# facebookresearch/dmc-net

Measured on AMD Instinct MI355X. Metric: clips/sec (3-seg 224x224) DMC-gen+ResNet-18 train step, higher is better.
Workload: dtype f32

## Files before the change

dmc-net_amd/csrc/bn_act.hip:

```cpp
#include "dmc_common.h"

using namespace dmc;

namespace {

constexpr int MAX_SPLIT = BN_MAX_SPLIT;

struct BnArgs {
    const float* x;
    const float* res;
    const float* gamma;
    const float* beta;
    const float* stats;
    const float* dy;
    float* y;
    float* dx;
    float* dres;
    int M, C, relu;
    unsigned char* mask;
    const float* keep;
    int hw;
    float slope;
};

template <int MODE>
__global__ __launch_bounds__(256) void bn_partial_kernel(BnArgs a, double* __restrict__ scratch) {
    __shared__ double sm[2][256][4];
    const int cq = a.C >> 2;
    const int tx = threadIdx.x % cq, ty = threadIdx.x / cq, rows = 256 / cq;
    const int per = (a.M + (int)gridDim.x - 1) / (int)gridDim.x;
    const int r0 = blockIdx.x * per, r1 = (r0 + per < a.M) ? r0 + per : a.M;
    float4 s0 = make_float4(0.f, 0.f, 0.f, 0.f), s1 = s0;
    float4 mean = s0, istd = s0, g = s0, b = s0;
    if (MODE == 1) {
        mean = reinterpret_cast<const float4*>(a.stats)[tx];
        istd = reinterpret_cast<const float4*>(a.stats + a.C)[tx];
        g = reinterpret_cast<const float4*>(a.gamma)[tx];
        b = reinterpret_cast<const float4*>(a.beta)[tx];
    }
// ... 356 lines not shown
                                                           int M, int C, int hw, float slope) {
    const int cq = C >> 2;
    const size_t total = (size_t)M * cq;
    for (size_t o = (size_t)blockIdx.x * 256 + threadIdx.x; o < total; o += (size_t)gridDim.x * 256) {
        const int tx = (int)(o % cq);
        const float4 x = reinterpret_cast<const float4*>(z)[o];
        float4 d = reinterpret_cast<const float4*>(dz)[o];
        float4 k = make_float4(1.f, 1.f, 1.f, 1.f);
        if (keep) k = reinterpret_cast<const float4*>(keep)[(size_t)((o / cq) / hw) * cq + tx];
        d.x *= k.x * (x.x > 0.f ? 1.f : slope); d.y *= k.y * (x.y > 0.f ? 1.f : slope);
        d.z *= k.z * (x.z > 0.f ? 1.f : slope); d.w *= k.w * (x.w > 0.f ? 1.f : slope);
        reinterpret_cast<float4*>(dx)[o] = d;
    }
}

__global__ __launch_bounds__(256) void channel_sum_final_kernel(const double* __restrict__ scratch,
                                                                float* __restrict__ out, int C, int split) {
    const int c = blockIdx.x * 8 + (threadIdx.x >> 5), sub = threadIdx.x & 31;
    double s, ss;
    reduce_partials(scratch, C, c, split, sub, s, ss);
    if (c < C && sub == 0) out[c] = (float)s;
}

bool shape_ok(int M, int C) {
    const int cq = C / 4;
    return M > 0 && C > 0 && C % 4 == 0 && cq <= 256 && 256 % cq == 0;
}

int split_of(int M, int C) {
    long sp = (long)M * C / 8192;
    return sp < 1 ? 1 : (sp > MAX_SPLIT ? MAX_SPLIT : (int)sp);
}

int stream_blocks(size_t total) {
    size_t b = (total + 255) / 256;
    return (int)(b < 1 ? 1 : (b > 8192 ? 8192 : b));
}


__device__ __forceinline__ void load8(const float* p, size_t i8, float (&v)[8]) {
    const float4 a = reinterpret_cast<const float4*>(p)[2 * i8], b = reinterpret_cast<const float4*>(p)[2 * i8 + 1];
    v[0] = a.x; v[1] = a.y; v[2] = a.z; v[3] = a.w; v[4] = b.x; v[5] = b.y; v[6] = b.z; v[7] = b.w;
}
__device__ __forceinline__ void store8(float* p, size_t i8, const float (&v)[8]) {
    reinterpret_cast<float4*>(p)[2 * i8] = make_float4(v[0], v[1], v[2], v[3]);
    reinterpret_cast<float4*>(p)[2 * i8 + 1] = make_float4(v[4], v[5], v[6], v[7]);
}

__global__ __launch_bounds__(256) void bn_apply_fwd_x3s_kernel(BnArgs a, unsigned short* __restrict__ ys, int s2d_h, int s2d_w) {
    const int c8 = a.C >> 3;
    const size_t total = (size_t)a.M * c8;
    for (size_t o = (size_t)blockIdx.x * 256 + threadIdx.x; o < total; o += (size_t)gridDim.x * 256) {
        const int tx = (int)(o & (size_t)(c8 - 1));
        const size_t m = o / c8;
        float mean[8], istd[8], g[8], b[8], x[8], v[8];
        load8(a.stats, tx, mean); load8(a.stats + a.C, tx, istd); load8(a.gamma, tx, g); load8(a.beta, tx, b);
        load8(a.x, o, x);
#pragma unroll
        for (int e = 0; e < 8; ++e) v[e] = fmaf((x[e] - mean[e]) * istd[e], g[e], b[e]);
        if (a.res) {
            float rr[8];
            load8(a.res, o, rr);
#pragma unroll
            for (int e = 0; e < 8; ++e) v[e] += rr[e];
        }
        if (a.relu) {
// ... 24 lines not shown
                                                               const float* __restrict__ dbeta, float inv_count,
                                                               unsigned short* __restrict__ dxs) {
    const int c8 = a.C >> 3;
    const size_t total = (size_t)a.M * c8;
    for (size_t o = (size_t)blockIdx.x * 256 + threadIdx.x; o < total; o += (size_t)gridDim.x * 256) {
        const int tx = (int)(o & (size_t)(c8 - 1));
        const size_t m = o / c8;
        float mean[8], istd[8], g[8], b[8], dg[8], db[8], x[8], d[8], xh[8], r[8];
        load8(a.stats, tx, mean); load8(a.stats + a.C, tx, istd); load8(a.gamma, tx, g); load8(a.beta, tx, b);
        load8(dgamma, tx, dg); load8(dbeta, tx, db);
        load8(a.x, o, x); load8(a.dy, o, d);
#pragma unroll
        for (int e = 0; e < 8; ++e) xh[e] = (x[e] - mean[e]) * istd[e];
        if (a.relu && a.mask) {
            const unsigned mw = reinterpret_cast<const unsigned short*>(a.mask)[o];
            const unsigned mb = (mw & 15u) | ((mw >> 8) << 4);
#pragma unroll
            for (int e = 0; e < 8; ++e) d[e] = ((mb >> e) & 1u) ? d[e] : 0.f;
        } else if (a.relu) {
            float rr[8];
            if (a.res) load8(a.res, o, rr);
#pragma unroll
            for (int e = 0; e < 8; ++e) {
                float v = fmaf(xh[e], g[e], b[e]);
                if (a.res) v += rr[e];
                d[e] = v > 0.f ? d[e] : 0.f;
            }
        }
        if (a.dres) store8(a.dres, o, d);
#pragma unroll
        for (int e = 0; e < 8; ++e) r[e] = g[e] * istd[e] * (d[e] - db[e] * inv_count - xh[e] * dg[e] * inv_count);
        if (a.dx) store8(a.dx, o, r);
        if (dxs) x3s_store8(dxs, r, (size_t)a.M, a.C >> 4, m, tx);
    }
}

__global__ __launch_bounds__(256) void pool_fwd_x3s_kernel(PoolArgs a, unsigned short* __restrict__ ys, unsigned* __restrict__ codes,
                                                           float* __restrict__ xmax) {
    const int c8 = a.C >> 3;
    const size_t total = (size_t)a.N * a.PH * a.PW * c8;
    for (size_t o = (size_t)blockIdx.x * 256 + threadIdx.x; o < total; o += (size_t)gridDim.x * 256) {
        const int tx = (int)(o & (size_t)(c8 - 1));
        size_t r = o / c8;
        const size_t mp = r;
        const int px = (int)(r % a.PW); r /= a.PW;
        const int py = (int)(r % a.PH);
        const int n = (int)(r / a.PH);
        float mean[8], istd[8], g[8], b[8], mx[8];
        load8(a.stats, tx, mean); load8(a.stats + a.C, tx, istd); load8(a.gamma, tx, g); load8(a.beta, tx, b);
        float xv[9][8];
#pragma unroll
        for (int k = 0; k < 9; ++k) {
            int iy = 2 * py + k / 3 - 1, ix = 2 * px + k % 3 - 1;
            iy = iy < 0 ? 0 : (iy >= a.H ? a.H - 1 : iy);
            ix = ix < 0 ? 0 : (ix >= a.W ? a.W - 1 : ix);
            load8(a.x, ((size_t)(n * a.H + iy) * a.W + ix) * c8 + tx, xv[k]);
        }
        if (codes) {
            float bx[8];
            unsigned ck[8];
#pragma unroll
            for (int e = 0; e < 8; ++e) { mx[e] = -INFINITY; bx[e] = 0.f; ck[e] = 0; }
#pragma unroll
            for (int k = 0; k < 9; ++k) {
                const int iy = 2 * py + k / 3 - 1, ix = 2 * px + k % 3 - 1;
                const bool in = iy >= 0 && iy < a.H && ix >= 0 && ix < a.W;
#pragma unroll
                for (int e = 0; e < 8; ++e) {
                    const float v = fmaxf(fmaf((xv[k][e] - mean[e]) * istd[e], g[e], b[e]), 0.f);
                    const bool take = in && v > mx[e];
                    mx[e] = take ? v : mx[e];
                    bx[e] = take ? xv[k][e] : bx[e];
                    ck[e] = take ? (unsigned)k : ck[e];
                }
            }
            reinterpret_cast<uint2*>(codes)[o] = make_uint2(ck[0] | (ck[1] << 8) | (ck[2] << 16) | (ck[3] << 24),
                                                            ck[4] | (ck[5] << 8) | (ck[6] << 16) | (ck[7] << 24));
            store8(xmax, o, bx);
        } else {
#pragma unroll
            for (int e = 0; e < 8; ++e) mx[e] = 0.f;
#pragma unroll
            for (int k = 0; k < 9; ++k)
#pragma unroll
                for (int e = 0; e < 8; ++e) mx[e] = fmaxf(mx[e], fmaxf(fmaf((xv[k][e] - mean[e]) * istd[e], g[e], b[e]), 0.f));
        }
        if (a.ypool) store8(a.ypool, o, mx);
        if (ys) x3s_store8(ys, mx, (size_t)a.N * a.PH * a.PW, a.C >> 4, mp, tx);
    }
}

bool shape_ok8(int M, int C) { return shape_ok(M, C) && C % 16 == 0 && C >= 16; }

}

extern "C" {

int dmc_bn_act_supported(int M, int C) { return shape_ok(M, C) ? 1 : 0; }

size_t dmc_bn_act_stats_bytes(int C) { return (((size_t)2 * C * sizeof(float)) + 15) / 16 * 16; }
size_t dmc_bn_act_scratch_bytes(int C) { return (size_t)MAX_SPLIT * C * 2 * sizeof(double); }

int dmc_bn_act_fwd(const float* x, const float* residual, const float* gamma, const float* beta,
                   float* running_mean, float* running_var, float* y, float* stats, void* scratch_,
                   unsigned char* relu_mask, int M, int C, int relu, int training, float eps,
                   float momentum, dmc_stream_t stream) {
    if (!x || !gamma || !beta || !running_mean || !running_var || !y || !stats || (training && !scratch_))
        return fail(DMC_E_INVALID, "dmc_bn_act_fwd: null pointer");
    if (!shape_ok(M, C)) return fail(DMC_E_INVALID, "dmc_bn_act_fwd: unsupported shape M=%d C=%d", M, C);
    hipStream_t s = (hipStream_t)stream;
    BnArgs a = {x, residual, gamma, beta, stats, nullptr, y, nullptr, nullptr, M, C, relu, relu_mask};
    double* scratch = static_cast<double*>(scratch_);
    int rc;
    const int split = split_of(M, C);
    if (training) {
        bn_partial_kernel<0><<<split, 256, 0, s>>>(a, scratch);
        if ((rc = check_launch("bn_partial"))) return rc;
    }
    bn_stats_final_kernel<<<(C + 7) / 8, 256, 0, s>>>(scratch, stats, running_mean, running_var, C,
                                                       (long)M, training, eps, momentum, split);
    if ((rc = check_launch("bn_stats_final"))) return rc;
    bn_apply_fwd_kernel<<<stream_blocks((size_t)M * (C / 4)), 256, 0, s>>>(a);
    return check_launch("bn_apply_fwd");
}

int dmc_bn_act_bwd(const float* x, const float* residual, const float* gamma, const float* beta,
                   const float* stats, void* scratch_, const float* dy, float* dx, float* dresidual,
                   float* dgamma, float* dbeta, const unsigned char* relu_mask, int M, int C, int relu,
                   dmc_stream_t stream) {
    if (!x || !gamma || !beta || !stats || !scratch_ || !dy || !dx || !dgamma || !dbeta)
        return fail(DMC_E_INVALID, "dmc_bn_act_bwd: null pointer");
    if (!shape_ok(M, C)) return fail(DMC_E_INVALID, "dmc_bn_act_bwd: unsupported shape M=%d C=%d", M, C);
    hipStream_t s = (hipStream_t)stream;
    BnArgs a = {x, residual, gamma, beta, stats, dy, nullptr, dx, dresidual, M, C, relu,
                const_cast<unsigned char*>(relu_mask)};
    double* scratch = static_cast<double*>(scratch_);
    int rc;
    const int split = split_of(M, C);
    bn_partial_kernel<1><<<split, 256, 0, s>>>(a, scratch);
    if ((rc = check_launch("bn_bwd_partial"))) return rc;
    bn_bwd_final_kernel<<<C, 256, 0, s>>>(scratch, dgamma, dbeta, C, split);
    if ((rc = check_launch("bn_bwd_final"))) return rc;
    bn_apply_bwd_kernel<<<stream_blocks((size_t)M * (C / 4)), 256, 0, s>>>(a, dgamma, dbeta, 1.f / (float)M);
    return check_launch("bn_apply_bwd");
}

int dmc_bn_relu_pool_supported(int N, int H, int W, int C) {
    return N > 0 && H > 0 && W > 0 && shape_ok(1, C) && C / 4 <= 64 ? 1 : 0;
}

int dmc_bn_relu_pool_fwd(const float* x, const float* gamma, const float* beta, float* running_mean,
                         float* running_var, float* y_pool, float* stats, void* scratch_, int N, int H,
                         int W, int C, int training, float eps, float momentum, dmc_stream_t stream) {
    if (!x || !gamma || !beta || !running_mean || !running_var || !y_pool || !stats || (training && !scratch_))
        return fail(DMC_E_INVALID, "dmc_bn_relu_pool_fwd: null pointer");
    if (!dmc_bn_relu_pool_supported(N, H, W, C))
        return fail(DMC_E_INVALID, "dmc_bn_relu_pool_fwd: unsupported shape N=%d H=%d W=%d C=%d", N, H, W, C);
    hipStream_t s = (hipStream_t)stream;
    const int M = N * H * W;
    BnArgs a = {x, nullptr, gamma, beta, stats, nullptr, nullptr, nullptr, nullptr, M, C, 1, nullptr};
    double* scratch = static_cast<double*>(scratch_);
    int rc;
    const int split = split_of(M, C);
    if (training) {
        bn_partial_kernel<0><<<split, 256, 0, s>>>(a, scratch);
        if ((rc = check_launch("bn_partial"))) return rc;
    }
    bn_stats_final_kernel<<<(C + 7) / 8, 256, 0, s>>>(scratch, stats, running_mean, running_var, C,
                                                       (long)M, training, eps, momentum, split);
    if ((rc = check_launch("bn_stats_final"))) return rc;
    PoolArgs p = {x, gamma, beta, stats, nullptr, y_pool, nullptr, N, H, W, C, (H - 1) / 2 + 1, (W - 1) / 2 + 1};
    pool_fwd_kernel<<<stream_blocks((size_t)N * p.PH * p.PW * (C / 4)), 256, 0, s>>>(p);
// ... 78 lines not shown
    return check_launch("channel_sum_final");
}

int dmc_bn_apply_act_x3s(const float* x, const float* residual, const float* gamma, const float* beta, const float* stats,
                         float* y, void* ys, unsigned char* relu_mask, int M, int C, int relu, dmc_stream_t stream) {
    if (!x || !gamma || !beta || !stats || (!y && !ys)) return fail(DMC_E_INVALID, "dmc_bn_apply_act_x3s: null pointer");
    if (!shape_ok8(M, C)) return fail(DMC_E_INVALID, "dmc_bn_apply_act_x3s: unsupported shape M=%d C=%d", M, C);
    BnArgs a = {x, residual, gamma, beta, stats, nullptr, y, nullptr, nullptr, M, C, relu, relu_mask};
    bn_apply_fwd_x3s_kernel<<<stream_blocks((size_t)M * (C / 8)), 256, 0, (hipStream_t)stream>>>(a, static_cast<unsigned short*>(ys), 0, 0);
    return check_launch("bn_apply_act_x3s");
}

int dmc_bn_apply_act_x3q(const float* x, const float* residual, const float* gamma, const float* beta, const float* stats,
                         float* y, void* yq, unsigned char* relu_mask, int N, int H, int W, int C, int relu, dmc_stream_t stream) {
    if (!x || !gamma || !beta || !stats || !yq) return fail(DMC_E_INVALID, "dmc_bn_apply_act_x3q: null pointer");
    if (N <= 0 || H <= 0 || W <= 0 || (H & 1) || (W & 1) || (long)N * H * W >= (1L << 31)) return fail(DMC_E_INVALID, "dmc_bn_apply_act_x3q: bad geometry");
    const int M = N * H * W;
    if (!shape_ok8(M, C)) return fail(DMC_E_INVALID, "dmc_bn_apply_act_x3q: unsupported shape M=%d C=%d", M, C);
    BnArgs a = {x, residual, gamma, beta, stats, nullptr, y, nullptr, nullptr, M, C, relu, relu_mask};
    bn_apply_fwd_x3s_kernel<<<stream_blocks((size_t)M * (C / 8)), 256, 0, (hipStream_t)stream>>>(a, static_cast<unsigned short*>(yq), H, W);
    return check_launch("bn_apply_act_x3q");
}

int dmc_bn_act_bwd_x3s(const float* x, const float* residual, const float* gamma, const float* beta, const float* stats,
                       void* scratch_, const float* dy, float* dx, void* dxs, float* dresidual, float* dgamma, float* dbeta,
                       const unsigned char* relu_mask, int M, int C, int relu, dmc_stream_t stream) {
    if (!x || !gamma || !beta || !stats || !scratch_ || !dy || (!dx && !dxs) || !dgamma || !dbeta)
        return fail(DMC_E_INVALID, "dmc_bn_act_bwd_x3s: null pointer");
    if (!shape_ok8(M, C)) return fail(DMC_E_INVALID, "dmc_bn_act_bwd_x3s: unsupported shape M=%d C=%d", M, C);
    hipStream_t s = (hipStream_t)stream;
    BnArgs a = {x, residual, gamma, beta, stats, dy, nullptr, dx, dresidual, M, C, relu, const_cast<unsigned char*>(relu_mask)};
    double* scratch = static_cast<double*>(scratch_);
    int rc;
    const int split = split_of(M, C);
    bn_partial_kernel<1><<<split, 256, 0, s>>>(a, scratch);
    if ((rc = check_launch("bn_bwd_partial"))) return rc;
    bn_bwd_final_kernel<<<C, 256, 0, s>>>(scratch, dgamma, dbeta, C, split);
    if ((rc = check_launch("bn_bwd_final"))) return rc;
    bn_apply_bwd_x3s_kernel<<<stream_blocks((size_t)M * (C / 8)), 256, 0, s>>>(a, dgamma, dbeta, 1.f / (float)M, static_cast<unsigned short*>(dxs));
    return check_launch("bn_apply_bwd_x3s");
}

int dmc_bn_relu_pool_fwd_arg(const float* x, const float* gamma, const float* beta, float* running_mean, float* running_var,
                             float* y_pool, void* ys, void* codes, float* xmax, float* stats, void* scratch_, int stat_split,
                             int N, int H, int W, int C, int training, float eps, float momentum, dmc_stream_t stream) {
    if (!x || !gamma || !beta || !running_mean || !running_var || (!y_pool && !ys) || !stats || (training && !scratch_))
        return fail(DMC_E_INVALID, "dmc_bn_relu_pool_fwd_x3s: null pointer");
    if (stat_split < 0 || stat_split > MAX_SPLIT) return fail(DMC_E_INVALID, "dmc_bn_relu_pool_fwd_arg: bad stat_split %d", stat_split);
    if ((codes == nullptr) != (xmax == nullptr)) return fail(DMC_E_INVALID, "dmc_bn_relu_pool_fwd_arg: codes and xmax go together");
    if (!dmc_bn_relu_pool_supported(N, H, W, C) || C % 16 != 0)
        return fail(DMC_E_INVALID, "dmc_bn_relu_pool_fwd_x3s: unsupported shape N=%d H=%d W=%d C=%d", N, H, W, C);
    hipStream_t s = (hipStream_t)stream;
    const int M = N * H * W;
    BnArgs a = {x, nullptr, gamma, beta, stats, nullptr, nullptr, nullptr, nullptr, M, C, 1, nullptr};
    double* scratch = static_cast<double*>(scratch_);
    int rc;
    const int split = stat_split > 0 ? stat_split : split_of(M, C);
    if (training && stat_split == 0) {
        bn_partial_kernel<0><<<split, 256, 0, s>>>(a, scratch);
        if ((rc = check_launch("bn_partial"))) return rc;
    }
    bn_stats_final_kernel<<<(C + 7) / 8, 256, 0, s>>>(scratch, stats, running_mean, running_var, C, (long)M, training, eps, momentum, split);
    if ((rc = check_launch("bn_stats_final"))) return rc;
    PoolArgs p = {x, gamma, beta, stats, nullptr, y_pool, nullptr, N, H, W, C, (H - 1) / 2 + 1, (W - 1) / 2 + 1};
    pool_fwd_x3s_kernel<<<stream_blocks((size_t)N * p.PH * p.PW * (C / 8)), 256, 0, s>>>(p, static_cast<unsigned short*>(ys),
                                                                                         static_cast<unsigned*>(codes), xmax);
    return check_launch("pool_fwd_x3s");
}

int dmc_bn_relu_pool_fwd_x3s(const float* x, const float* gamma, const float* beta, float* running_mean, float* running_var,
                             float* y_pool, void* ys, float* stats, void* scratch_, int N, int H, int W, int C, int training,
                             float eps, float momentum, dmc_stream_t stream) {
    return dmc_bn_relu_pool_fwd_arg(x, gamma, beta, running_mean, running_var, y_pool, ys, nullptr, nullptr, stats, scratch_, 0, N, H, W, C,
                                    training, eps, momentum, stream);
}

int dmc_bn_relu_pool_bwd_arg(const float* x, const float* gamma, const float* beta, const float* stats, void* scratch_,
                             const float* d_pool, const void* codes, const float* xmax, float* dx, float* dgamma, float* dbeta,
                             int N, int H, int W, int C, dmc_stream_t stream) {
    if (!x || !gamma || !beta || !stats || !scratch_ || !d_pool || !codes || !xmax || !dx || !dgamma || !dbeta)
        return fail(DMC_E_INVALID, "dmc_bn_relu_pool_bwd_arg: null pointer");
    if (!dmc_bn_relu_pool_supported(N, H, W, C) || C % 16 != 0)
        return fail(DMC_E_INVALID, "dmc_bn_relu_pool_bwd_arg: unsupported shape N=%d H=%d W=%d C=%d", N, H, W, C);
    hipStream_t s = (hipStream_t)stream;
    PoolArgs p = {x, gamma, beta, stats, d_pool, nullptr, dx, N, H, W, C, (H - 1) / 2 + 1, (W - 1) / 2 + 1};
    double* scratch = static_cast<double*>(scratch_);
    const int MP = N * p.PH * p.PW;
    BnArgs a = {xmax, nullptr, gamma, beta, stats, d_pool, nullptr, nullptr, nullptr, MP, C, 1, nullptr};
    const int split = split_of(MP, C);
    int rc;
    bn_partial_kernel<1><<<split, 256, 0, s>>>(a, scratch);
    if ((rc = check_launch("pool_bwd_sums"))) return rc;
    bn_bwd_final_kernel<<<C, 256, 0, s>>>(scratch, dgamma, dbeta, C, split);
    if ((rc = check_launch("bn_bwd_final"))) return rc;
    const long tiles = (long)N * ((p.PH + PT - 1) / PT) * ((p.PW + PT - 1) / PT);
    const long blocks = tiles * 4 > 8192 ? 8192 : tiles * 4;
    pool_bwd_kernel<2><<<(int)blocks, 256, 0, s>>>(p, nullptr, dgamma, dbeta, 1.f / (float)((long)N * H * W),
                                                   const_cast<unsigned*>(static_cast<const unsigned*>(codes)));
    return check_launch("pool_bwd_apply");
}

int dmc_bn_act_bwd_x3s_apply(const float* x, const float* residual, const float* gamma, const float* beta, const float* stats,
                             const float* dy, float* dx, void* dxs, float* dresidual, const float* dgamma, const float* dbeta,
                             const unsigned char* relu_mask, int M, int C, int relu, dmc_stream_t stream) {
    if (!x || !gamma || !beta || !stats || !dy || (!dx && !dxs) || !dgamma || !dbeta)
        return fail(DMC_E_INVALID, "dmc_bn_act_bwd_x3s_apply: null pointer");
    if (!shape_ok8(M, C)) return fail(DMC_E_INVALID, "dmc_bn_act_bwd_x3s_apply: unsupported shape M=%d C=%d", M, C);
    BnArgs a = {x, residual, gamma, beta, stats, dy, nullptr, dx, dresidual, M, C, relu, const_cast<unsigned char*>(relu_mask)};
    bn_apply_bwd_x3s_kernel<<<stream_blocks((size_t)M * (C / 8)), 256, 0, (hipStream_t)stream>>>(a, dgamma, dbeta, 1.f / (float)M, static_cast<unsigned short*>(dxs));
    return check_launch("bn_apply_bwd_x3s");
}

}
```

dmc-net_amd/csrc/conv_x3q.hip:

```cpp
#include "dmc_common.h"
#include "x3s_common.h"
#include <type_traits>
#include <utility>

using namespace dmc;
using namespace dmc::x3;

namespace {

constexpr int QBM = 256, QBN = 64;
constexpr int QWSLOT = 3 * QBN * 32;
constexpr int QWB = 3 * QWSLOT;
constexpr int QEP = 272, QETILE = 32 * QEP;

template <int NW_, int NPB_, int NT_>
struct QG {
    static constexpr int NW = NW_, NPB = NPB_, NT = NT_;
    static constexpr int NA = NW / 2;
    static constexpr int KP = (NT + NA - 1) / NA;
    static constexpr int PT = 3 * KP;
    static constexpr int KW = (18 + NA - 1) / NA;
    static constexpr int ZROW = 32 * NT;
    static constexpr int PSL = (ZROW + 1) * 32;
    static constexpr int PB = 3 * PSL;
// ... 715 lines not shown
    }
    float* out = a.part + (size_t)blockIdx.y * a.Cout * a.Cin;
    const int ci = tci * 64 + 32 * wj + l31;
#pragma unroll
    for (int e = 0; e < 16; ++e) {
        const int co = tco * 64 + 32 * wi + 8 * (e >> 2) + 4 * khalf + (e & 3);
        out[(size_t)co * a.Cin + ci] = acc[e];
    }
}

__global__ __launch_bounds__(256) void x3q_wgrad_reduce_kernel(const float* __restrict__ part, float* __restrict__ dw, int ngroup, long numel) {
    __shared__ float4 red[16][17];
    const int o = threadIdx.x & 15, sl = threadIdx.x >> 4;
    for (long i0 = (long)blockIdx.x * 64; i0 < numel; i0 += (long)gridDim.x * 64) {
        const long i = i0 + 4 * o;
        float4 s = make_float4(0.f, 0.f, 0.f, 0.f);
        if (i < numel)
            for (int k = sl; k < ngroup; k += 16) {
                const float4 v = *reinterpret_cast<const float4*>(part + (size_t)k * numel + i);
                s.x += v.x; s.y += v.y; s.z += v.z; s.w += v.w;
            }
        red[sl][o] = s;
        __syncthreads();
        if (sl == 0 && i < numel) {
            float4 t = red[0][o];
#pragma unroll
            for (int k = 1; k < 16; ++k) { const float4 v = red[k][o]; t.x += v.x; t.y += v.y; t.z += v.z; t.w += v.w; }
            *reinterpret_cast<float4*>(dw + i) = t;
        }
        __syncthreads();
    }
}

struct QWgPlan { int R, HP, steps, tiles, groups, per_group, steps1, groups1, per_group1; };
bool q_wgrad_plan(int N, int OH, int OW, int Cin, int Cout, QWgPlan& p) {
    if (Cin % 64 != 0 || Cout % 64 != 0 || N <= 0) return false;
    if (OW == 28 && OH == 28) { p.R = 1; p.HP = 29; }
    else if (OW == 14 && OH == 14) { p.R = 2; p.HP = 16; }
    else if (OW == 7 && OH == 7) { p.R = 4; p.HP = 8; }
    else return false;
    p.steps = N * p.HP / p.R;
    p.tiles = (Cout / 64) * (Cin / 64);
    int groups = 256 / p.tiles;
    if (groups < 1) groups = 1;
    if (groups > p.steps) groups = p.steps;
    p.per_group = (p.steps + groups - 1) / groups;
    p.groups = (p.steps + p.per_group - 1) / p.per_group;
    const long Mq = (long)N * OH * OW;
    p.steps1 = (int)((Mq + W1PX - 1) / W1PX);
    int g1 = 512 / p.tiles;
    if (g1 < 1) g1 = 1;
    if (g1 > p.steps1) g1 = p.steps1;
    p.per_group1 = (p.steps1 + g1 - 1) / g1;
    p.groups1 = (p.steps1 + p.per_group1 - 1) / p.per_group1;
    return true;
}

template <int OW_, int R, int HP_>
int launch_q_wgrad(const QWgPlan& p, const X3qWgArgs& a, hipStream_t s) {
    using G = QWgGeom<OW_, R, HP_>;
    static_assert(G::LDS <= 160 * 1024, "weight-gradient tiles exceed the LDS");
    static LdsLimit lim;
    const hipError_t attr = lim.raise(reinterpret_cast<const void*>(&x3q_wgrad_kernel<OW_, R, HP_>), G::LDS);
    if (attr != hipSuccess) return fail(DMC_E_LAUNCH, "x3q_wgrad: cannot raise the dynamic LDS limit: %s", hipGetErrorString(attr));
    x3q_wgrad_kernel<OW_, R, HP_><<<dim3(p.tiles, p.groups), 768, G::LDS, s>>>(a);
    return check_launch("x3q_wgrad");
// ... 88 lines not shown
    a.pps0 = a.pps1 = Cout / 16;
    const int var = q_variant(a.M, OW, Cin);
    return var == 0 ? launch_q<ProgDgrad, 2, QGBig>(a, (hipStream_t)stream) : var == 1 ? launch_q<ProgDgrad, 1, QGBig>(a, (hipStream_t)stream)
                                                                                        : launch_q<ProgDgrad, 2, QGTwo>(a, (hipStream_t)stream);
}

int dmc_x3q_conv_wgrad_supported(int N, int OH, int OW, int Cin, int Cout) {
    QWgPlan p;
    return q_shape_ok(N, OH, OW, Cin, Cout) && q_wgrad_plan(N, OH, OW, Cin, Cout, p) ? 1 : 0;
}

size_t dmc_x3q_conv_wgrad_bytes(int N, int OH, int OW, int Cin, int Cout) {
    QWgPlan p;
    if (!q_wgrad_plan(N, OH, OW, Cin, Cout, p)) return 0;
    return ((size_t)p.groups * 9 + (size_t)p.groups1) * Cout * Cin * sizeof(float);
}

int dmc_x3q_conv_wgrad(const void* xq, const void* dys3, const void* dys1, float* dw3, float* dw1, float* workspace, int N, int OH,
                       int OW, int Cin, int Cout, dmc_stream_t stream) {
    QWgPlan p;
    if (!xq || !dys3 || !dys1 || !dw3 || !dw1 || !workspace) return fail(DMC_E_INVALID, "dmc_x3q_conv_wgrad: null pointer");
    if (!dmc_x3q_conv_wgrad_supported(N, OH, OW, Cin, Cout) || !q_wgrad_plan(N, OH, OW, Cin, Cout, p))
        return fail(DMC_E_INVALID, "dmc_x3q_conv_wgrad: unsupported shape N=%d OH=%d OW=%d Cin=%d Cout=%d", N, OH, OW, Cin, Cout);
    hipStream_t s = (hipStream_t)stream;
    const long Mq = (long)N * OH * OW;
    X3qWgArgs a;
    a.xq = xq; a.dys = dys3; a.part = workspace;
    a.N = N; a.OH = OH; a.Cin = Cin; a.Cout = Cout;
    a.plane_bytes = (unsigned)Mq * 32u;
    a.steps = p.steps; a.per_group = p.per_group; a.tiles_ci = Cin / 64;
    int rc = OW == 28 ? launch_q_wgrad<28, 1, 29>(p, a, s) : OW == 14 ? launch_q_wgrad<14, 2, 16>(p, a, s) : launch_q_wgrad<7, 4, 8>(p, a, s);
    if (rc) return rc;
    const long numel3 = (long)Cout * 9 * Cin, numel1 = (long)Cout * Cin;
    long blocks = (numel3 + 63) / 64;
    x3q_wgrad_reduce_kernel<<<(int)(blocks > 4096 ? 4096 : blocks), 256, 0, s>>>(workspace, dw3, p.groups, numel3);
    rc = check_launch("x3q_wgrad_reduce");
    if (rc) return rc;
    float* part1 = workspace + (size_t)p.groups * numel3;
    X3qWg1Args b;
    b.xq = xq; b.dys = dys1; b.part = part1; b.Cin = Cin; b.Cout = Cout; b.Mq = Mq; b.plane_bytes = (unsigned)Mq * 32u;
    b.steps = p.steps1; b.per_group = p.per_group1; b.tiles_ci = Cin / 64;
    static LdsLimit lim1;
    const hipError_t attr = lim1.raise(reinterpret_cast<const void*>(&x3q_wgrad1_kernel), W1LDS);
    if (attr != hipSuccess) return fail(DMC_E_LAUNCH, "x3q_wgrad1: cannot raise the dynamic LDS limit: %s", hipGetErrorString(attr));
    x3q_wgrad1_kernel<<<dim3(p.tiles, p.groups1), 256, W1LDS, s>>>(b);
    rc = check_launch("x3q_wgrad1");
    if (rc) return rc;
    blocks = (numel1 + 63) / 64;
    x3q_wgrad_reduce_kernel<<<(int)(blocks > 4096 ? 4096 : blocks), 256, 0, s>>>(part1, dw1, p.groups1, numel1);
    return check_launch("x3q_wgrad_reduce1");
}

}
```

dmc-net_amd/csrc/conv_x3s.hip:

```cpp
#include "dmc_common.h"
#include "x3s_common.h"
#include <type_traits>

using namespace dmc;
using namespace dmc::x3;

namespace {

__global__ __launch_bounds__(256) void x3s_split_kernel(const float* __restrict__ x, unsigned short* __restrict__ xs, long M, int C) {
    const int c8 = C >> 3;
    const long total = M * c8;
    const int nchunk = C >> 4;
    for (long o = (long)blockIdx.x * 256 + threadIdx.x; o < total; o += (long)gridDim.x * 256) {
        const long m = o / c8;
        const int g = (int)(o - m * c8);
        const float4 a = reinterpret_cast<const float4*>(x)[2 * o], b = reinterpret_cast<const float4*>(x)[2 * o + 1];
        const float v[8] = {a.x, a.y, a.z, a.w, b.x, b.y, b.z, b.w};
        x3s_store8(xs, v, (size_t)M, nchunk, (size_t)m, g);
    }
}

__global__ __launch_bounds__(256) void x3s_merge_kernel(const unsigned short* __restrict__ xs, float* __restrict__ x, long M, int C) {
    const long total = M * C;
    const size_t plane = (size_t)M * 16;
// ... 667 lines not shown
    const int ci = tci * 64 + 32 * wj + l31;
#pragma unroll
    for (int t = 0; t < 3; ++t)
#pragma unroll
        for (int e = 0; e < 16; ++e) {
            const int co = tco * 64 + 32 * wi + 8 * (e >> 2) + 4 * khalf + (e & 3);
            out[((size_t)co * 9 + 3 * trow + t) * a.Cin + ci] = acc[t][e];
        }
}

__global__ __launch_bounds__(256) void x3s_wgrad_reduce_kernel(const float* __restrict__ part, float* __restrict__ dw, int ngroup, long numel) {
    __shared__ float4 red[16][17];
    const int o = threadIdx.x & 15, sl = threadIdx.x >> 4;
    for (long i0 = (long)blockIdx.x * 64; i0 < numel; i0 += (long)gridDim.x * 64) {
        const long i = i0 + 4 * o;
        float4 s = make_float4(0.f, 0.f, 0.f, 0.f);
        if (i < numel)
            for (int k = sl; k < ngroup; k += 16) {
                const float4 v = *reinterpret_cast<const float4*>(part + (size_t)k * numel + i);
                s.x += v.x; s.y += v.y; s.z += v.z; s.w += v.w;
            }
        red[sl][o] = s;
        __syncthreads();
        if (sl == 0 && i < numel) {
            float4 t = red[0][o];
#pragma unroll
            for (int k = 1; k < 16; ++k) { const float4 v = red[k][o]; t.x += v.x; t.y += v.y; t.z += v.z; t.w += v.w; }
            *reinterpret_cast<float4*>(dw + i) = t;
        }
        __syncthreads();
    }
}

struct X3WgPlan { int R, steps, tiles, groups, per_group; };
bool x3s_wgrad_plan(int N, int H, int W, int Cin, int Cout, X3WgPlan& p) {
    p.R = W == 56 ? 1 : W == 28 ? 2 : W == 14 ? 4 : W == 7 ? 9 : 0;
    if (!p.R || (H + 2) % p.R != 0 || (W == 7 && H != 7) || Cin % 64 != 0 || Cout % 64 != 0) return false;
    p.steps = N * (H + 2) / p.R;
    p.tiles = (Cout / 64) * (Cin / 64);
    int groups = 256 / p.tiles;
    if (groups < 1) groups = 1;
    if (groups > p.steps) groups = p.steps;
    p.per_group = (p.steps + groups - 1) / groups;
    p.groups = (p.steps + p.per_group - 1) / p.per_group;
    return true;
}

template <int W_, int R>
int launch_x3s_wgrad(const X3WgPlan& p, X3WgArgs a, float* dw, hipStream_t s) {
    using G = WgGeom<W_, R>;
    static_assert(G::LDS <= 160 * 1024, "weight-gradient tiles exceed the LDS");
    static LdsLimit lim_attr;
    const hipError_t attr = lim_attr.raise(reinterpret_cast<const void*>(&x3s_wgrad_kernel<W_, R>), G::LDS);
    if (attr != hipSuccess) return fail(DMC_E_LAUNCH, "x3s_wgrad: cannot raise the dynamic LDS limit: %s", hipGetErrorString(attr));
    x3s_wgrad_kernel<W_, R><<<dim3(p.tiles, p.groups), 768, G::LDS, s>>>(a);
    int rc = check_launch("x3s_wgrad");
    if (rc || p.groups == 1) return rc;
    const long numel = (long)a.Cout * 9 * a.Cin;
    const long blocks = (numel + 63) / 64;
    x3s_wgrad_reduce_kernel<<<(int)(blocks > 4096 ? 4096 : blocks), 256, 0, s>>>(a.part, dw, p.groups, numel);
    return check_launch("x3s_wgrad_reduce");
}

__global__ __launch_bounds__(256) void x3s_bnb_final_kernel(const double* __restrict__ part, int nblk, int C,
                                                            float* __restrict__ dgamma, float* __restrict__ dbeta) {
    __shared__ double red[2][4];
    const int c = blockIdx.x, lane = threadIdx.x & 63, wave = threadIdx.x >> 6;
    double s = 0.0, ss = 0.0;
    for (int b = threadIdx.x; b < nblk; b += 256) {
        const double2 v = *reinterpret_cast<const double2*>(part + ((size_t)b * C + c) * 2);
        s += v.x;
        ss += v.y;
    }
#pragma unroll
    for (int o = 32; o > 0; o >>= 1) { s += __shfl_down(s, o, 64); ss += __shfl_down(ss, o, 64); }
    if (lane == 0) { red[0][wave] = s; red[1][wave] = ss; }
    __syncthreads();
    if (threadIdx.x != 0) return;
    dbeta[c] = (float)(red[0][0] + red[0][1] + red[0][2] + red[0][3]);
    dgamma[c] = (float)(red[1][0] + red[1][1] + red[1][2] + red[1][3]);
}

int stream_blocks(long total) {
    long b = (total + 255) / 256;
    return (int)(b < 1 ? 1 : (b > 8192 ? 8192 : b));
}

}

extern "C" {

size_t dmc_x3s_slices_bytes(long M, int C) { return (size_t)M * (size_t)C * 6; }

// ... 152 lines not shown
```

dmc-net_amd/csrc/x3s_common.h:

```cpp
#pragma once
#include "dmc_common.h"

namespace dmc {
namespace x3 {

typedef float f32x16 __attribute__((ext_vector_type(16)));
typedef __bf16 bf16x8 __attribute__((ext_vector_type(8)));
typedef unsigned u32x4 __attribute__((ext_vector_type(4)));
typedef const __attribute__((address_space(3))) char* lds_cptr;

__device__ __forceinline__ f32x16 mfma_bf16(const u32x4& a, const u32x4& b, const f32x16& c) {
    return __builtin_amdgcn_mfma_f32_32x32x16_bf16(__builtin_bit_cast(bf16x8, a), __builtin_bit_cast(bf16x8, b), c, 0, 0, 0);
}

__device__ __forceinline__ void split3(float v, unsigned& u0, unsigned& u1, unsigned& u2) {
    u0 = __float_as_uint(v);
    const float r1 = v - __uint_as_float(u0 & 0xffff0000u);
    u1 = __float_as_uint(r1);
    u2 = __float_as_uint(r1 - __uint_as_float(u1 & 0xffff0000u));
}
__device__ __forceinline__ unsigned pack_hi(unsigned hi_of_second, unsigned hi_of_first) {
    return __builtin_amdgcn_perm(hi_of_second, hi_of_first, 0x07060302u);
}

// ... 22 lines not shown
    f[0] = ua[0]; f[1] = ua[1]; f[2] = ub[0]; f[3] = ub[1];
}

constexpr unsigned NOPIX = 0x40000000u;

struct WgGroupPos { int n, y; };
__device__ __forceinline__ WgGroupPos wg_group_at(int q, int R, int HP) {
    const int g = R * q, n = g / HP;
    WgGroupPos p;
    p.n = __builtin_amdgcn_readfirstlane(n);
    p.y = __builtin_amdgcn_readfirstlane(g - n * HP);
    return p;
}
__device__ __forceinline__ WgGroupPos wg_group_next(WgGroupPos p, int R, int HP) {
    p.y += R;
    if (p.y >= HP) { p.y -= HP; ++p.n; }
    return p;
}
__device__ __forceinline__ WgGroupPos wg_group_prev(WgGroupPos p, int R, int HP) {
    p.y -= R;
    if (p.y < 0) { p.y += HP; --p.n; }
    return p;
}
__device__ __forceinline__ void wg_group_base(const WgGroupPos& p, int N, int W, unsigned img_bytes, unsigned& tbase, unsigned& img_off) {
    const bool in = p.n >= 0 && p.n < N;
    tbase = in ? (unsigned)((p.y - 1) * W) * 32u : NOPIX;
    img_off = in ? (unsigned)p.n * img_bytes : 0u;
}
__device__ __forceinline__ unsigned wg_lane_off(unsigned tbase, unsigned pre, unsigned img_bytes) {
    const unsigned t = tbase + pre;
    return t < img_bytes ? t : OOB;
}

typedef float f32x4 __attribute__((ext_vector_type(4)));
__device__ __forceinline__ f32x4 mfma16(const u32x4& a, const u32x4& b, const f32x4& c) {
    return __builtin_amdgcn_mfma_f32_16x16x32_bf16(__builtin_bit_cast(bf16x8, a), __builtin_bit_cast(bf16x8, b), c, 0, 0, 0);
}

__device__ __forceinline__ void split8(const float4& lo, const float4& hi, u32x4& s0, u32x4& s1, u32x4& s2) {
    const float v[8] = {lo.x, lo.y, lo.z, lo.w, hi.x, hi.y, hi.z, hi.w};
    unsigned u0[8], u1[8], u2[8];
#pragma unroll
    for (int e = 0; e < 8; ++e) split3(v[e], u0[e], u1[e], u2[e]);
#pragma unroll
    for (int e = 0; e < 4; ++e) {
        s0[e] = pack_hi(u0[2 * e + 1], u0[2 * e]);
        s1[e] = pack_hi(u1[2 * e + 1], u1[2 * e]);
        s2[e] = pack_hi(u2[2 * e + 1], u2[2 * e]);
    }
}

}
}
```

Before: 3550.

## Add vectorized BN backward partial-sum kernel and few-group wgrad reduce kernel

Adds a BN backward partial reduction kernel that reads 8 channels per thread with 4-row unrolling, templated on mask, sign or residual ReLU gating. It reduces within each block through shared memory and picks its split count from the row batching. It is used for the wide BN backward, x3s BN backward and pool backward paths. It also adds a wgrad reduce kernel for fewer than 16 groups, which spreads the group dimension across thread slots and finishes with a shared-memory column sum. Both aim for better memory parallelism in reductions that were latency- or occupancy-bound, at the cost of more kernel variants and extra shared-memory traffic.

Result: no change. 3562, median of 6 (+0.3%).

```diff
diff --git a/dmc-net_amd/csrc/bn_act.hip b/dmc-net_amd/csrc/bn_act.hip
--- a/dmc-net_amd/csrc/bn_act.hip
+++ b/dmc-net_amd/csrc/bn_act.hip
@@ -5,6 +5,7 @@
 namespace {
 
 constexpr int MAX_SPLIT = BN_MAX_SPLIT;
+constexpr int P8_ROWS = 4;
 
 struct BnArgs {
     const float* x;
@@ -427,6 +428,12 @@
     return sp < 1 ? 1 : (sp > MAX_SPLIT ? MAX_SPLIT : (int)sp);
 }
 
+int split8_of(int M, int C, int cap) {
+    const int batch = P8_ROWS * (2048 / C), nbatch = (M + batch - 1) / batch;
+    const int k = (nbatch + cap - 1) / cap;
+    return (nbatch + k - 1) / k;
+}
+
 int stream_blocks(size_t total) {
     size_t b = (total + 255) / 256;
     return (int)(b < 1 ? 1 : (b > 8192 ? 8192 : b));
@@ -517,6 +524,66 @@
         for (int e = 0; e < 8; ++e) r[e] = g[e] * istd[e] * (d[e] - db[e] * inv_count - xh[e] * dg[e] * inv_count);
         if (a.dx) store8(a.dx, o, r);
         if (dxs) x3s_store8(dxs, r, (size_t)a.M, a.C >> 4, m, tx);
+    }
+}
+
+template <int SIGN>
+__global__ __launch_bounds__(256) void bn_partial_bwd_x3s_kernel(BnArgs a, double* __restrict__ scratch) {
+    __shared__ float sm[256][16];
+    const int c8 = a.C >> 3;
+    const int tx = threadIdx.x % c8, ty = threadIdx.x / c8, rows = 256 / c8;
+    const int batch = P8_ROWS * rows, nbatch = (a.M + batch - 1) / batch;
+    const long per = (long)batch * ((nbatch + (int)gridDim.x - 1) / (int)gridDim.x);
+    const long r0 = (long)blockIdx.x * per, r1 = (r0 + per < a.M) ? r0 + per : a.M;
+    const bool by_mask = SIGN == 0 && a.relu && a.mask;
+    constexpr bool by_sign = SIGN > 0, with_res = SIGN == 2;
+    float mean[8], istd[8], g[8], b[8], s0[8], s1[8];
+    load8(a.stats, tx, mean); load8(a.stats + a.C, tx, istd); load8(a.gamma, tx, g); load8(a.beta, tx, b);
+#pragma unroll
+    for (int e = 0; e < 8; ++e) s0[e] = s1[e] = 0.f;
+    for (long r = r0 + ty; r < r1; r += (long)P8_ROWS * rows) {
+        float x[P8_ROWS][8], d[P8_ROWS][8], rr[with_res ? P8_ROWS : 1][8];
+        unsigned mw[P8_ROWS];
+        bool ok[P8_ROWS];
+#pragma unroll
+        for (int u = 0; u < P8_ROWS; ++u) {
+            const long ru = r + (long)u * rows;
+            ok[u] = ru < r1;
+            const size_t o = (size_t)(ok[u] ? ru : r) * c8 + tx;
+            load8(a.x, o, x[u]); load8(a.dy, o, d[u]);
+            mw[u] = by_mask ? reinterpret_cast<const unsigned short*>(a.mask)[o] : 0u;
+            if (with_res) load8(a.res, o, rr[u]);
+        }
+#pragma unroll
+        for (int u = 0; u < P8_ROWS; ++u) {
+            const unsigned mb = (mw[u] & 15u) | ((mw[u] >> 8) << 4);
+#pragma unroll
+            for (int e = 0; e < 8; ++e) {
+                const float xh = (x[u][e] - mean[e]) * istd[e];
+                bool keep = ok[u];
+                if (by_mask) keep = keep && ((mb >> e) & 1u);
+                if (by_sign) {
+                    float v = fmaf(xh, g[e], b[e]);
+                    if (with_res) v += rr[with_res ? u : 0][e];
+                    keep = keep && v > 0.f;
+                }
+                const float dz = keep ? d[u][e] : 0.f;
+                s0[e] += dz;
+                s1[e] = fmaf(dz, xh, s1[e]);
+            }
+        }
+    }
+#pragma unroll
+    for (int e = 0; e < 8; ++e) { sm[threadIdx.x][e] = s0[e]; sm[threadIdx.x][8 + e] = s1[e]; }
+    __syncthreads();
+    for (int c = threadIdx.x; c < a.C; c += 256) {
+        const int col = c >> 3, e = c & 7;
+        double acc0 = 0.0, acc1 = 0.0;
+        for (int t = 0; t < rows; ++t) {
+            acc0 += (double)sm[t * c8 + col][e];
+            acc1 += (double)sm[t * c8 + col][8 + e];
+        }
+        reinterpret_cast<double2*>(scratch)[(size_t)c * MAX_SPLIT + blockIdx.x] = make_double2(acc0, acc1);
     }
 }
 
@@ -576,6 +643,15 @@
 }
 
 bool shape_ok8(int M, int C) { return shape_ok(M, C) && C % 16 == 0 && C >= 16; }
+
+int launch_partial_bwd_x3s(const BnArgs& a, double* scratch, hipStream_t s) {
+    const bool by_mask = !a.relu || a.mask;
+    const int split = split8_of(a.M, a.C, by_mask ? MAX_SPLIT : 768);
+    if (by_mask) bn_partial_bwd_x3s_kernel<0><<<split, 256, 0, s>>>(a, scratch);
+    else if (!a.res) bn_partial_bwd_x3s_kernel<1><<<split, 256, 0, s>>>(a, scratch);
+    else bn_partial_bwd_x3s_kernel<2><<<split, 256, 0, s>>>(a, scratch);
+    return split;
+}
 
 }
 
@@ -621,8 +697,10 @@
                 const_cast<unsigned char*>(relu_mask)};
     double* scratch = static_cast<double*>(scratch_);
     int rc;
-    const int split = split_of(M, C);
-    bn_partial_kernel<1><<<split, 256, 0, s>>>(a, scratch);
+    const bool wide = shape_ok8(M, C) && (reinterpret_cast<size_t>(relu_mask) & 1) == 0;
+    int split = split_of(M, C);
+    if (wide) split = launch_partial_bwd_x3s(a, scratch, s);
+    else bn_partial_kernel<1><<<split, 256, 0, s>>>(a, scratch);
     if ((rc = check_launch("bn_bwd_partial"))) return rc;
     bn_bwd_final_kernel<<<C, 256, 0, s>>>(scratch, dgamma, dbeta, C, split);
     if ((rc = check_launch("bn_bwd_final"))) return rc;
@@ -767,8 +845,7 @@
     BnArgs a = {x, residual, gamma, beta, stats, dy, nullptr, dx, dresidual, M, C, relu, const_cast<unsigned char*>(relu_mask)};
     double* scratch = static_cast<double*>(scratch_);
     int rc;
-    const int split = split_of(M, C);
-    bn_partial_kernel<1><<<split, 256, 0, s>>>(a, scratch);
+    const int split = launch_partial_bwd_x3s(a, scratch, s);
     if ((rc = check_launch("bn_bwd_partial"))) return rc;
     bn_bwd_final_kernel<<<C, 256, 0, s>>>(scratch, dgamma, dbeta, C, split);
     if ((rc = check_launch("bn_bwd_final"))) return rc;
@@ -822,9 +899,8 @@
     double* scratch = static_cast<double*>(scratch_);
     const int MP = N * p.PH * p.PW;
     BnArgs a = {xmax, nullptr, gamma, beta, stats, d_pool, nullptr, nullptr, nullptr, MP, C, 1, nullptr};
-    const int split = split_of(MP, C);
     int rc;
-    bn_partial_kernel<1><<<split, 256, 0, s>>>(a, scratch);
+    const int split = launch_partial_bwd_x3s(a, scratch, s);
     if ((rc = check_launch("pool_bwd_sums"))) return rc;
     bn_bwd_final_kernel<<<C, 256, 0, s>>>(scratch, dgamma, dbeta, C, split);
     if ((rc = check_launch("bn_bwd_final"))) return rc;
diff --git a/dmc-net_amd/csrc/conv_x3q.hip b/dmc-net_amd/csrc/conv_x3q.hip
--- a/dmc-net_amd/csrc/conv_x3q.hip
+++ b/dmc-net_amd/csrc/conv_x3q.hip
@@ -771,6 +771,16 @@
     }
 }
 
+__global__ __launch_bounds__(256) void x3q_wgrad_reduce_few_kernel(const float* __restrict__ part, float* __restrict__ dw, int ngroup, long numel) {
+    __shared__ float4 red[16][64];
+    wgrad_reduce_body<64, 1>(part, dw, ngroup, numel, red);
+}
+void launch_x3q_wgrad_reduce(const float* part, float* dw, int ngroup, long numel, hipStream_t s) {
+    const long blocks = (numel + 63) / 64;
+    if (ngroup < 16) x3q_wgrad_reduce_few_kernel<<<wgrad_reduce_blocks(numel, 64), 256, 0, s>>>(part, dw, ngroup, numel);
+    else x3q_wgrad_reduce_kernel<<<(int)(blocks > 4096 ? 4096 : blocks), 256, 0, s>>>(part, dw, ngroup, numel);
+}
+
 struct QWgPlan { int R, HP, steps, tiles, groups, per_group, steps1, groups1, per_group1; };
 bool q_wgrad_plan(int N, int OH, int OW, int Cin, int Cout, QWgPlan& p) {
     if (Cin % 64 != 0 || Cout % 64 != 0 || N <= 0) return false;
@@ -925,8 +935,7 @@
     int rc = OW == 28 ? launch_q_wgrad<28, 1, 29>(p, a, s) : OW == 14 ? launch_q_wgrad<14, 2, 16>(p, a, s) : launch_q_wgrad<7, 4, 8>(p, a, s);
     if (rc) return rc;
     const long numel3 = (long)Cout * 9 * Cin, numel1 = (long)Cout * Cin;
-    long blocks = (numel3 + 63) / 64;
-    x3q_wgrad_reduce_kernel<<<(int)(blocks > 4096 ? 4096 : blocks), 256, 0, s>>>(workspace, dw3, p.groups, numel3);
+    launch_x3q_wgrad_reduce(workspace, dw3, p.groups, numel3, s);
     rc = check_launch("x3q_wgrad_reduce");
     if (rc) return rc;
     float* part1 = workspace + (size_t)p.groups * numel3;
@@ -939,8 +948,7 @@
     x3q_wgrad1_kernel<<<dim3(p.tiles, p.groups1), 256, W1LDS, s>>>(b);
     rc = check_launch("x3q_wgrad1");
     if (rc) return rc;
-    blocks = (numel1 + 63) / 64;
-    x3q_wgrad_reduce_kernel<<<(int)(blocks > 4096 ? 4096 : blocks), 256, 0, s>>>(part1, dw1, p.groups1, numel1);
+    launch_x3q_wgrad_reduce(part1, dw1, p.groups1, numel1, s);
     return check_launch("x3q_wgrad_reduce1");
 }
 
diff --git a/dmc-net_amd/csrc/conv_x3s.hip b/dmc-net_amd/csrc/conv_x3s.hip
--- a/dmc-net_amd/csrc/conv_x3s.hip
+++ b/dmc-net_amd/csrc/conv_x3s.hip
@@ -723,6 +723,16 @@
     }
 }
 
+__global__ __launch_bounds__(256) void x3s_wgrad_reduce_few_kernel(const float* __restrict__ part, float* __restrict__ dw, int ngroup, long numel) {
+    __shared__ float4 red[16][64];
+    wgrad_reduce_body<64, 1>(part, dw, ngroup, numel, red);
+}
+void launch_x3s_wgrad_reduce(const float* part, float* dw, int ngroup, long numel, hipStream_t s) {
+    const long blocks = (numel + 63) / 64;
+    if (ngroup < 16) x3s_wgrad_reduce_few_kernel<<<wgrad_reduce_blocks(numel, 64), 256, 0, s>>>(part, dw, ngroup, numel);
+    else x3s_wgrad_reduce_kernel<<<(int)(blocks > 4096 ? 4096 : blocks), 256, 0, s>>>(part, dw, ngroup, numel);
+}
+
 struct X3WgPlan { int R, steps, tiles, groups, per_group; };
 bool x3s_wgrad_plan(int N, int H, int W, int Cin, int Cout, X3WgPlan& p) {
     p.R = W == 56 ? 1 : W == 28 ? 2 : W == 14 ? 4 : W == 7 ? 9 : 0;
@@ -748,8 +758,7 @@
     int rc = check_launch("x3s_wgrad");
     if (rc || p.groups == 1) return rc;
     const long numel = (long)a.Cout * 9 * a.Cin;
-    const long blocks = (numel + 63) / 64;
-    x3s_wgrad_reduce_kernel<<<(int)(blocks > 4096 ? 4096 : blocks), 256, 0, s>>>(a.part, dw, p.groups, numel);
+    launch_x3s_wgrad_reduce(a.part, dw, p.groups, numel, s);
     return check_launch("x3s_wgrad_reduce");
 }
 
diff --git a/dmc-net_amd/csrc/x3s_common.h b/dmc-net_amd/csrc/x3s_common.h
--- a/dmc-net_amd/csrc/x3s_common.h
+++ b/dmc-net_amd/csrc/x3s_common.h
@@ -78,6 +78,51 @@
     return t < img_bytes ? t : OOB;
 }
 
+template <int COLS, int UNR>
+__device__ __forceinline__ void wgrad_reduce_body(const float* __restrict__ part, float* __restrict__ dw, int ngroup, long numel,
+                                                  float4 (*red)[COLS]) {
+    constexpr int SLOTS = 4 * (64 / COLS), LPT = 16 / SLOTS;
+    const int o = (int)threadIdx.x % COLS;
+    const int slot = ((int)threadIdx.x >> 6) * (64 / COLS) + ((int)threadIdx.x & 63) / COLS;
+    for (long i0 = (long)blockIdx.x * (4 * COLS); i0 < numel; i0 += (long)gridDim.x * (4 * COLS)) {
+        const long i = i0 + 4 * o;
+        float4 s[LPT];
+#pragma unroll
+        for (int j = 0; j < LPT; ++j) s[j] = make_float4(0.f, 0.f, 0.f, 0.f);
+        if (i < numel)
+            for (int kb = 0; kb < ngroup; kb += 16 * UNR) {
+                float4 v[UNR][LPT];
+#pragma unroll
+                for (int u = 0; u < UNR; ++u)
+#pragma unroll
+                    for (int j = 0; j < LPT; ++j) {
+                        const int k = kb + 16 * u + slot + SLOTS * j;
+                        v[u][j] = make_float4(0.f, 0.f, 0.f, 0.f);
+                        if (k < ngroup) v[u][j] = *reinterpret_cast<const float4*>(part + (size_t)k * numel + i);
+                    }
+#pragma unroll
+                for (int u = 0; u < UNR; ++u)
+#pragma unroll
+                    for (int j = 0; j < LPT; ++j) { s[j].x += v[u][j].x; s[j].y += v[u][j].y; s[j].z += v[u][j].z; s[j].w += v[u][j].w; }
+            }
+#pragma unroll
+        for (int j = 0; j < LPT; ++j) red[slot + SLOTS * j][o] = s[j];
+        __syncthreads();
+        if ((int)threadIdx.x < 4 * COLS && i0 + (long)threadIdx.x < numel) {
+            const float* col = reinterpret_cast<const float*>(red) + threadIdx.x;
+            float t = col[0];
+#pragma unroll
+            for (int k = 1; k < 16; ++k) t += col[k * 4 * COLS];
+            dw[i0 + threadIdx.x] = t;
+        }
+        __syncthreads();
+    }
+}
+inline int wgrad_reduce_blocks(long numel, int cols) {
+    const long b = (numel + 4 * cols - 1) / (4 * cols);
+    return (int)(b > 16384 ? 16384 : b);
+}
+
 typedef float f32x4 __attribute__((ext_vector_type(4)));
 __device__ __forceinline__ f32x4 mfma16(const u32x4& a, const u32x4& b, const f32x4& c) {
     return __builtin_amdgcn_mfma_f32_16x16x32_bf16(__builtin_bit_cast(bf16x8, a), __builtin_bit_cast(bf16x8, b), c, 0, 0, 0);
```
